# shehryar-malik/icrl

Measured on AMD Instinct MI355X. Metric: env-steps/sec (ICRL outer loop, HCWithPos-v0), higher is better.
Workload: dtype f32

## Files before the change

### icrl_amd/csrc/rollout.hip

```cpp
#include <stdio.h>
#include <stdlib.h>

#include "common.h"
#include "cost_fn.h"
#include "generic.h"

namespace icrl {

__global__ void policy_transpose_kernel(PolLayout L, const float* __restrict__ p, float* __restrict__ pt) {
  for (int i = blockIdx.x * blockDim.x + threadIdx.x; i < L.n; i += gridDim.x * blockDim.x) {
    int dst = i;
    for (int w = 0; w < 3; ++w) {
      if (i >= L.W1[w] && i < L.b1[w]) { int r = i - L.W1[w]; int j = r / L.O, k = r % L.O; dst = L.W1[w] + k * L.H1 + j; }
      if (i >= L.W2[w] && i < L.b2[w]) { int r = i - L.W2[w]; int j = r / L.H1, k = r % L.H1; dst = L.W2[w] + k * L.H2 + j; }
    }
    if (i >= L.Wa && i < L.ba) { int r = i - L.Wa; int a = r / L.H2, j = r % L.H2; dst = L.Wa + j * L.A + a; }
    pt[dst] = p[i];
  }
}

__global__ void costnet_transpose_kernel(CnLayout L, const float* __restrict__ p, float* __restrict__ pt) {
  for (int i = blockIdx.x * blockDim.x + threadIdx.x; i < L.n; i += gridDim.x * blockDim.x) {
    int dst = i;
    if (i >= L.W0 && i < L.b0) { int r = i - L.W0; int j = r / L.in, k = r % L.in; dst = L.W0 + k * L.H1 + j; }
// ... 10 lines not shown
  alignas(16) float x[MAX_OBS];
  alignas(16) float h[3][MAX_H];
  alignas(16) float g[3][MAX_H];
  alignas(16) float cx[MAX_CN_IN];
  alignas(16) float ch[2][MAX_H];
  float act_raw[MAX_ACT];
  float act_clip[MAX_ACT];
  float scal[4];
};

template <int OCT, int CIT>
struct WaveRegs {
  static constexpr int NA = 16 * (OCT > CIT ? OCT : CIT);
  union { float w1[NA]; float c0[NA]; };
  union { float w2[MAX_H]; float c1[MAX_H]; };
  float wh[MAX_H];
  union { float b1; float cb0; };
  union { float b2; float cb1; };
  union { float bh; float cbo; };
  union { float ls; float co; };
  float sd, lsd, i2v;
  int sel[(16 * (CIT > 0 ? CIT : 1) + WAVE - 1) / WAVE];
};
template <int OCT> using PolRegs = WaveRegs<OCT, 0>;
template <int CIT> using CnRegs = WaveRegs<0, CIT>;

template <int OCT, class Regs>
__device__ __forceinline__ void load_pol_regs(const PolLayout& L, const float* __restrict__ PT, Regs& R) {
  const int lane = threadIdx.x & 63;
  const int w = __builtin_amdgcn_readfirstlane(threadIdx.x >> 6);
  const int j1 = lane < L.H1 ? lane : 0, j2 = lane < L.H2 ? lane : 0;
#pragma unroll
  for (int k = 0; k < 16 * OCT; ++k) R.w1[k] = (w < 3 && k < L.O) ? PT[L.W1[w] + k * L.H1 + j1] : 0.f;
#pragma unroll
  for (int k = 0; k < MAX_H; ++k) R.w2[k] = (w < 3 && k < L.H1) ? PT[L.W2[w] + k * L.H2 + j2] : 0.f;
  R.b1 = w < 3 ? PT[L.b1[w] + j1] : 0.f;
  R.b2 = w < 3 ? PT[L.b2[w] + j2] : 0.f;
  R.bh = 0.f; R.ls = 0.f; R.sd = 1.f; R.lsd = 0.f; R.i2v = 2.f;
  if (w == 0) {
    const int a = lane < L.A ? lane : 0;
#pragma unroll
    for (int j = 0; j < MAX_H; ++j) R.wh[j] = j < L.H2 ? PT[L.Wa + j * L.A + a] : 0.f;
    R.bh = PT[L.ba + a];
    if (!L.discrete) R.ls = PT[L.log_std + a];
    R.sd = expf(R.ls); R.lsd = logf(R.sd); R.i2v = 2.f * (R.sd * R.sd);
  } else if (w < 3) {
#pragma unroll
    for (int j = 1; j < MAX_H; ++j) R.wh[j] = 0.f;
    R.wh[0] = PT[(w == 1 ? L.Wv : L.Wc) + j2];
    R.bh = PT[w == 1 ? L.bv : L.bc];
  }
}

template <int OCT, class Regs>
__device__ __forceinline__ void policy_forward_block(const PolLayout& L, const Regs& R, ActShared& sh,
                                                     const float* noise_row, int deterministic,
                                                     const float* alow, const float* ahigh,
                                                     const float* given = nullptr ) {
  const int lane = threadIdx.x & 63;
  const int w = __builtin_amdgcn_readfirstlane(threadIdx.x >> 6);
  if (w < 3) {
    f32x4 xs[4 * OCT];
#pragma unroll
    for (int i = 0; i < 4 * OCT; ++i) xs[i] = *reinterpret_cast<const f32x4*>(&sh.x[4 * i]);
    float acc = 0.f;
#pragma unroll
    for (int k = 0; k < 16 * OCT; ++k) acc = fmaf(R.w1[k], xs[k >> 2][k & 3], acc);
    sh.h[w][lane] = lane < L.H1 ? fast_tanh(acc + R.b1) : 0.f;
  }
  __syncthreads();
  if (w < 3) {
    f32x4 hs[MAX_H / 4];
#pragma unroll
    for (int i = 0; i < MAX_H / 4; ++i) hs[i] = *reinterpret_cast<const f32x4*>(&sh.h[w][4 * i]);
    float acc = 0.f;
#pragma unroll
    for (int k = 0; k < MAX_H; ++k) acc = fmaf(R.w2[k], hs[k >> 2][k & 3], acc);
    sh.g[w][lane] = lane < L.H2 ? fast_tanh(acc + R.b2) : 0.f;
  }
  __syncthreads();
  if (w == 0) {
    float mean = 0.f;
    {
      f32x4 gs[MAX_H / 4];
#pragma unroll
      for (int i = 0; i < MAX_H / 4; ++i) gs[i] = *reinterpret_cast<const f32x4*>(&sh.g[0][4 * i]);
      float acc = 0.f;
#pragma unroll
      for (int j = 0; j < MAX_H; ++j) acc = fmaf(R.wh[j], gs[j >> 2][j & 3], acc);
      mean = acc + R.bh;
    }
    if (!L.discrete) {
      float lp = 0.f, entl = 0.f;
      if (lane < L.A) {
        const float std = R.sd;
        float act = mean;
        if (given != nullptr) act = given[lane];
        else if (!deterministic) act = mean + noise_row[lane] * std;
        const float diff = act - mean;
        lp = -(diff * diff) / R.i2v - R.lsd - LOG_SQRT_2PI_F;
        entl = HALF_LOG_2PI_PLUS_HALF_F + R.lsd;
        sh.act_raw[lane] = act;
        float c = act;
        if (alow != nullptr && ahigh != nullptr) c = fminf(fmaxf(act, alow[lane]), ahigh[lane]);
        sh.act_clip[lane] = c;
      }
      lp = wave_sum_fast(lp);
      const float ent = wave_sum_fast(entl);
      if (lane == 0) { sh.scal[2] = lp; sh.scal[3] = ent; }
    } else {
      float m = wave_max(lane < L.A ? mean : -INFINITY);
      float e = lane < L.A ? expf(mean - m) : 0.f;
      float lse = m + logf(wave_sum(e));
      float logp = mean - lse;
      float p = lane < L.A ? expf(logp) : 0.f;
      float cdf = 0.f;
      int action = 0;
      if (given != nullptr) {
        action = (int)given[0];
      } else if (deterministic) {
        float best = wave_max(lane < L.A ? p : -1.f);
        unsigned long long ball = __ballot(lane < L.A && p == best);
        action = __ffsll((long long)ball) - 1;
      } else {
        const float u = noise_row[0];
        int cnt = 0;
        for (int a = 0; a < L.A; ++a) {
          cdf += __shfl(p, a, 64);
          cnt += (u >= cdf) ? 1 : 0;
        }
        action = cnt < L.A - 1 ? cnt : L.A - 1;
      }
      const float lp = __shfl(logp, action, 64);
// ... 618 lines not shown
    const int d = a.dones[n];
    if (d) nm.ret[n] = 0.0;
    if (has_cost) {
      double c = (double)a.raw_cost[n];
      if (nm.norm_cost) c = fmin(fmax(c / cden, -nm.clip_cost), nm.clip_cost);
      if (a.cost_out) a.cost_out[n] = c;
      if (a.cost_f32) a.cost_f32[n] = (float)c;
      if (d) nm.cost_ret[n] = 0.0;
    }
    if (a.last_dones) a.last_dones[n] = (uint8_t)d;
  }
}

__device__ __forceinline__ double np_pairwise_sum_wave(const double* a, int n) {
  const int leaves = n >> 7;
  if ((n & 127) != 0 || (leaves & (leaves - 1)) != 0 || leaves > 8) return np_pairwise_sum(a, n);
  const int lane = threadIdx.x & 63;
  const int L = lane >> 3, k = lane & 7;
  const double* p = a + 128 * (L < leaves ? L : 0) + k;
  double v[16];
#pragma unroll
  for (int i = 0; i < 16; ++i) v[i] = p[8 * i];
  double r = v[0];
#pragma unroll
  for (int i = 1; i < 16; ++i) r += v[i];
  r += __shfl_xor(r, 1, 64);
  r += __shfl_xor(r, 2, 64);
  r += __shfl_xor(r, 4, 64);
  if (leaves >= 2) r += __shfl_xor(r, 8, 64);
  if (leaves >= 4) r += __shfl_xor(r, 16, 64);
  if (leaves >= 8) r += __shfl_xor(r, 32, 64);
  return __shfl(r, 0, 64);
}

__device__ __forceinline__ double np_leaf_sum_wave(const double* a, int n) {
  const int lane = threadIdx.x & 63;
  if (n < 8) {
    double r = 0.0;
    for (int i = 0; i < n; ++i) r += a[i];
    return r;
  }
  double r = 0.0;
  if (lane < 8) {
    r = a[lane];
    for (int i = 8; i < n - (n % 8); i += 8) r += a[i + lane];
  }
  const double r0 = __shfl(r, 0, 64), r1 = __shfl(r, 1, 64), r2 = __shfl(r, 2, 64), r3 = __shfl(r, 3, 64);
  const double r4 = __shfl(r, 4, 64), r5 = __shfl(r, 5, 64), r6 = __shfl(r, 6, 64), r7 = __shfl(r, 7, 64);
  double res = ((r0 + r1) + (r2 + r3)) + ((r4 + r5) + (r6 + r7));
  for (int i = n - (n % 8); i < n; ++i) res += a[i];
  return res;
}

__device__ __forceinline__ void column_moments(const double* col, int stride, int N, double& bm, double& bv) {
  auto load16 = [&](int r0, double (&v)[16]) {
#pragma unroll
    for (int k = 0; k < 16; ++k) v[k] = col[(r0 + k < N ? r0 + k : N - 1) * stride];
  };
  double va[16], vb[16];
  double sum = 0.0;
  load16(0, va);
  for (int r0 = 0; r0 < N; r0 += 32) {
    load16(r0 + 16 < N ? r0 + 16 : 0, vb);
    __builtin_amdgcn_sched_barrier(0);
#pragma unroll
    for (int k = 0; k < 16; ++k) if (r0 + k < N) sum += va[k];
    load16(r0 + 32 < N ? r0 + 32 : 0, va);
    __builtin_amdgcn_sched_barrier(0);
#pragma unroll
    for (int k = 0; k < 16; ++k) if (r0 + 16 + k < N) sum += vb[k];
  }
  bm = sum / (double)N;
  double sq = 0.0;
  for (int r0 = 0; r0 < N; r0 += 32) {
    load16(r0 + 16 < N ? r0 + 16 : 0, vb);
#pragma unroll
    for (int k = 0; k < 16; ++k) { const double d = va[k] - bm; va[k] = d * d; }
    __builtin_amdgcn_sched_barrier(0);
#pragma unroll
    for (int k = 0; k < 16; ++k) if (r0 + k < N) sq += va[k];
    load16(r0 + 32 < N ? r0 + 32 : 0, va);
#pragma unroll
    for (int k = 0; k < 16; ++k) { const double d = vb[k] - bm; vb[k] = d * d; }
    __builtin_amdgcn_sched_barrier(0);
#pragma unroll
    for (int k = 0; k < 16; ++k) if (r0 + 16 + k < N) sq += vb[k];
  }
  bv = sq / (double)N;
}

__device__ __forceinline__ void column_moments_contig(const double* col, int N, double& bm, double& bv) {
  double va[16], vb[16];
  double sum = 0.0;
  const int NF = N & ~31;
#pragma unroll
  for (int k = 0; k < 16; ++k) va[k] = col[k];
  int r0 = 0;
  for (; r0 < NF; r0 += 32) {
#pragma unroll
    for (int k = 0; k < 16; ++k) vb[k] = col[r0 + 16 + k];
    __builtin_amdgcn_sched_barrier(0);
#pragma unroll
    for (int k = 0; k < 16; ++k) sum += va[k];
#pragma unroll
    for (int k = 0; k < 16; ++k) va[k] = col[r0 + 32 + k];
    __builtin_amdgcn_sched_barrier(0);
#pragma unroll
    for (int k = 0; k < 16; ++k) sum += vb[k];
  }
  if (r0 < N) {
#pragma unroll
    for (int k = 0; k < 16; ++k) vb[k] = col[r0 + 16 + k];
#pragma unroll
    for (int k = 0; k < 16; ++k) if (r0 + k < N) sum += va[k];
#pragma unroll
    for (int k = 0; k < 16; ++k) if (r0 + 16 + k < N) sum += vb[k];
  }
  bm = sum / (double)N;
  double sq = 0.0;
#pragma unroll
  for (int k = 0; k < 16; ++k) va[k] = col[k];
  for (r0 = 0; r0 < NF; r0 += 32) {
#pragma unroll
    for (int k = 0; k < 16; ++k) vb[k] = col[r0 + 16 + k];
#pragma unroll
    for (int k = 0; k < 16; ++k) { const double d = va[k] - bm; va[k] = d * d; }
    __builtin_amdgcn_sched_barrier(0);
#pragma unroll
    for (int k = 0; k < 16; ++k) sq += va[k];
#pragma unroll
    for (int k = 0; k < 16; ++k) va[k] = col[r0 + 32 + k];
#pragma unroll
    for (int k = 0; k < 16; ++k) { const double d = vb[k] - bm; vb[k] = d * d; }
    __builtin_amdgcn_sched_barrier(0);
#pragma unroll
    for (int k = 0; k < 16; ++k) sq += vb[k];
  }
  if (r0 < N) {
#pragma unroll
    for (int k = 0; k < 16; ++k) vb[k] = col[r0 + 16 + k];
#pragma unroll
    for (int k = 0; k < 16; ++k) { const double d = va[k] - bm; va[k] = d * d; }
#pragma unroll
    for (int k = 0; k < 16; ++k) { const double d = vb[k] - bm; vb[k] = d * d; }
#pragma unroll
    for (int k = 0; k < 16; ++k) if (r0 + k < N) sq += va[k];
#pragma unroll
    for (int k = 0; k < 16; ++k) if (r0 + 16 + k < N) sq += vb[k];
  }
  bv = sq / (double)N;
}

__global__ void __launch_bounds__(1024) norm_step_small_kernel(NormStepArgs a) {
  __shared__ double chunk[NORM_CHUNK];
  __shared__ double vec[2][128], dev2[2][128];
  __shared__ double mean_s[MAX_OBS], var_s[MAX_OBS];
  __shared__ double dens[2];
  const int tid = threadIdx.x, nt = blockDim.x, lane = tid & 63, wv = tid >> 6;
  const int N = a.N, O = a.O;
  const icrl_norm_t& nm = a.nm;
  const bool has_cost = a.raw_cost != nullptr;
  for (int i = tid; i < N * O; i += nt) chunk[i] = a.raw_obs[i];
  if (tid < N) {
    double r = nm.ret[tid], c = has_cost ? nm.cost_ret[tid] : 0.0;
    if (nm.training) {
      r = r * nm.reward_gamma + a.raw_rew[tid];
      if (has_cost) c = c * nm.cost_gamma + (double)a.raw_cost[tid];
    }
    vec[0][tid] = r; vec[1][tid] = c;
  }
  double o_mean = 0.0, o_var = 1.0, o_cnt = 0.0;
  if (tid < O) { o_mean = nm.obs_mean[tid]; o_var = nm.obs_var[tid]; o_cnt = nm.obs_count[0]; }
  __syncthreads();
  if (nm.training) {
    if (tid < O) {
      double bm, bv;
      column_moments(chunk + tid, O, N, bm, bv);
      chan_merge(o_mean, o_var, o_cnt, bm, bv, (double)N);
      nm.obs_mean[tid] = o_mean; nm.obs_var[tid] = o_var;
      if (tid == 0) nm.obs_count[0] = (double)N + o_cnt;
    }
    if (wv == 15 || (wv == 14 && has_cost)) {
      const int v = wv == 15 ? 0 : 1;
      double* st = v == 0 ? nm.ret_stats : nm.cost_stats;
      const double bm = np_leaf_sum_wave(vec[v], N) / (double)N;
      for (int i = lane; i < N; i += 64) { const double d = vec[v][i] - bm; dev2[v][i] = d * d; }
      __builtin_amdgcn_wave_barrier();
      __builtin_amdgcn_s_waitcnt(0xC07F);
      const double bv = np_leaf_sum_wave(dev2[v], N) / (double)N;
      double m = st[0], var = st[1];
      const double cnt = st[2];
      chan_merge(m, var, cnt, bm, bv, (double)N);
      if (lane == 0) { st[0] = m; st[1] = var; st[2] = (double)N + cnt; }
      if (lane == 0) dens[v] = sqrt(var + nm.epsilon);
    }
  } else {
    if (tid == 0) { dens[0] = sqrt(nm.ret_stats[1] + nm.epsilon); dens[1] = sqrt(nm.cost_stats[1] + nm.epsilon); }
  }
  if (nm.training && !has_cost && tid == 0) dens[1] = sqrt(nm.cost_stats[1] + nm.epsilon);
  if (tid < O) { mean_s[tid] = o_mean; var_s[tid] = o_var; }
  __syncthreads();
  for (int idx = tid; idx < N * O; idx += nt) {
    const int j = idx % O;
    double o = chunk[idx];
    if (nm.norm_obs) o = fmin(fmax((o - mean_s[j]) / sqrt(var_s[j] + nm.epsilon), -nm.clip_obs), nm.clip_obs);
    if (a.obs_out) a.obs_out[idx] = o;
    if (a.obs_f32) a.obs_f32[idx] = (float)o;
  }
  if (tid < N) {
    const int n = tid;
    double r = a.raw_rew[n];
    if (nm.norm_reward) r = fmin(fmax(r / dens[0], -nm.clip_reward), nm.clip_reward);
    if (a.rew_out) a.rew_out[n] = r;
    if (a.rew_f32) a.rew_f32[n] = (float)r;
    const int d = a.dones[n];
    if (nm.training || d) nm.ret[n] = d ? 0.0 : vec[0][n];
    if (has_cost) {
      double c = (double)a.raw_cost[n];
      if (nm.norm_cost) c = fmin(fmax(c / dens[1], -nm.clip_cost), nm.clip_cost);
      if (a.cost_out) a.cost_out[n] = c;
      if (a.cost_f32) a.cost_f32[n] = (float)c;
      if (nm.training || d) nm.cost_ret[n] = d ? 0.0 : vec[1][n];
    }
    if (a.last_dones) a.last_dones[n] = (uint8_t)d;
  }
}

constexpr int NORM_MAX_N_TRACE = 1024;
__device__ unsigned long long g_rollout_prof[8];
__device__ unsigned long long g_rollout_prof_wide[16];
__device__ unsigned long long g_wide_trace[NORM_MAX_N_TRACE * 4];
__device__ __forceinline__ unsigned long long prof_now() {
  unsigned long long t;
  asm volatile("s_memtime %0\n\ts_waitcnt lgkmcnt(0)" : "=s"(t)::"memory");
  return t;
}

struct PersistArgs {
  ActStepArgs act;
  icrl_norm_t nm;
  int T;
  double* xch_obs;
  double* xch_rew;
  float* xch_cost;
  unsigned* xch_done;
  unsigned* counter;
  unsigned long long* xg;
  unsigned g_magic;
  int prof;
};

__device__ __forceinline__ void xstore(double* p, double v) {
  __hip_atomic_store(reinterpret_cast<unsigned long long*>(p), (unsigned long long)__double_as_longlong(v), __ATOMIC_RELAXED, __HIP_MEMORY_SCOPE_AGENT);
}
__device__ __forceinline__ void xstore(float* p, float v) {
  __hip_atomic_store(reinterpret_cast<unsigned*>(p), __float_as_uint(v), __ATOMIC_RELAXED, __HIP_MEMORY_SCOPE_AGENT);
}
__device__ __forceinline__ void xstore(unsigned* p, unsigned v) { __hip_atomic_store(p, v, __ATOMIC_RELAXED, __HIP_MEMORY_SCOPE_AGENT); }
__device__ __forceinline__ double xload(const double* p) {
  return __longlong_as_double((long long)__hip_atomic_load(reinterpret_cast<const unsigned long long*>(p), __ATOMIC_RELAXED, __HIP_MEMORY_SCOPE_AGENT));
}
__device__ __forceinline__ float xload(const float* p) {
  return __uint_as_float(__hip_atomic_load(reinterpret_cast<const unsigned*>(p), __ATOMIC_RELAXED, __HIP_MEMORY_SCOPE_AGENT));
}
__device__ __forceinline__ unsigned xload(const unsigned* p) { return __hip_atomic_load(p, __ATOMIC_RELAXED, __HIP_MEMORY_SCOPE_AGENT); }
__device__ __forceinline__ void gstore(unsigned long long* p, unsigned tag, unsigned payload) {
  __hip_atomic_store(p, ((unsigned long long)tag << 32) | (unsigned long long)payload, __ATOMIC_RELAXED, __HIP_MEMORY_SCOPE_AGENT);
}
__device__ __forceinline__ unsigned long long gload(const unsigned long long* p) {
  return __hip_atomic_load(p, __ATOMIC_RELAXED, __HIP_MEMORY_SCOPE_AGENT);
}

__device__ __forceinline__ void grid_barrier(unsigned* flags, int N, int n, unsigned value, int& spin_limit) {
  asm volatile("s_waitcnt vmcnt(0)" ::: "memory");
  __syncthreads();
  if (threadIdx.x < 64) {
    const int lane = threadIdx.x;
    if (lane == 0) xstore(flags + n, value);
    int spins = 0;
    bool ok = false;
    while (spins < spin_limit && !ok) {
      const unsigned v0 = lane < N ? xload(flags + lane) : value;
      const unsigned v1 = lane + 64 < N ? xload(flags + lane + 64) : value;
      ok = __all(v0 >= value && v1 >= value);
      ++spins;
    }
    if (!ok) spin_limit = 1;
  }
  __syncthreads();
}

constexpr int GRAN_MAX = 12;
constexpr int REC_MAX = GRAN_MAX / 2;

static inline size_t persist_dyn_lds(int N, int O, int A) { return ((size_t)O * (size_t)(N + 64) + (size_t)O * (size_t)A) * sizeof(double); }

template <int OCT, int CIT, bool GRAN, bool PROF = false, bool MON = false, bool POINT = true, bool DISC = false>
__device__ __forceinline__ void rollout_persistent_body(const PersistArgs& p) {
  extern __shared__ __attribute__((aligned(16))) double dyn_lds[];
  __shared__ ActShared sh;
  double* const chunk = dyn_lds;
  double* const Bl = dyn_lds + p.act.pl.O * (p.act.env.n_envs + 64);
  __shared__ double vec[2][128], dev2[2][128], ret_s[128], cret_s[128], rawr_s[128];
  __shared__ float rawc_s[128];
  __shared__ double dens[2];
  __shared__ float noise_s[MAX_ACT], alow_s[MAX_ACT], ahigh_s[MAX_ACT];
  __shared__ int done_s[128];
  __shared__ int last_done_s;
  const ActStepArgs& a = p.act;
  icrl_norm_t nm = p.nm; globalize(nm);
  icrl_buffer_t buf = a.buf; globalize(buf);
  icrl_agent_t ag = a.ag; globalize(ag);
  icrl_costnet_t cnet = a.cn; globalize(cnet);
  unsigned long long* const xg_all = as_global(p.xg);
  const float* const noise_g = as_global(a.noise);
  double* const raw_plane = MON ? as_global(a.raw_plane) : nullptr;
  WaveRegs<OCT, CIT> R;
  WaveRegs<OCT, CIT>& C = R;
  load_pol_regs<OCT>(a.pl, a.PT, R);
  if constexpr (CIT > 0) { if (threadIdx.x >= 192 && a.has_cn) load_cn_regs<CIT>(a.cn, a.cl, C); }
  const icrl_cost_fn_t cf = a.cf;
  const int n = blockIdx.x;
  const int tid = threadIdx.x, lane = tid & 63;
  const int w = __builtin_amdgcn_readfirstlane(tid >> 6);
  const int O = a.pl.O, A = a.pl.A, N = a.env.n_envs, T = p.T;
  const int AS = buf.act_store;
  const int NA = a.pl.discrete ? 1 : A;
  const int NP = N + 64;
  const int G = 2 * O + 4;
  const int R16 = O + 2;
  typedef unsigned int rec_u4 __attribute__((ext_vector_type(4)));
  const __amdgpu_buffer_rsrc_t xrs = __builtin_amdgcn_make_buffer_rsrc(xg_all, 0, 2 * N * G * 8, 0x00020000);
  auto rstore = [&](int byte_off, rec_u4 v) { __builtin_amdgcn_raw_buffer_store_b128(v, xrs, byte_off, 0, 16); };
  auto rload = [&](int byte_off) -> rec_u4 { return __builtin_amdgcn_raw_buffer_load_b128(xrs, byte_off, 0, 16); };
  for (int i = tid; i < O * NP; i += 256) chunk[i] = 0.0;
  const bool has_cost = a.has_cn != 0;
  const uint32_t e_key = a.env.key[n];
  uint32_t e_ctr = a.env.step_count[n];
  int e_tep = a.env.t_ep[n];
  icrl_env_t env = a.env; globalize(env);
  for (int i = tid; i < O * a.env.act_dim; i += 256) Bl[i] = a.env.B[i];
  env.B = Bl;
  const bool has_box = a.alow != nullptr && a.ahigh != nullptr;
  if (tid < MAX_ACT) { alow_s[tid] = (has_box && tid < A) ? a.alow[tid] : 0.f; ahigh_s[tid] = (has_box && tid < A) ? a.ahigh[tid] : 0.f; }
  for (int i = tid; i < MAX_OBS; i += 256) {
    sh.x[i] = i < O ? (float)ag.last_obs[(size_t)n * O + i] : 0.f;
    if (i < O) sh.s_old[i] = a.env.s[(size_t)n * O + i];
  }
  if (tid < N) { ret_s[tid] = nm.ret[tid]; cret_s[tid] = nm.cost_ret[tid]; }
  if (tid == 0) last_done_s = ag.last_dones[n];
  double o_mean = 0.0, o_var = 1.0, o_cnt = 0.0, o_last = 0.0;
  if (tid < O) { o_mean = nm.obs_mean[tid]; o_var = nm.obs_var[tid]; o_cnt = nm.obs_count[0]; o_last = ag.last_obs[(size_t)n * O + tid]; }
  double st_m = 0.0, st_v = 1.0, st_c = 0.0;
  if (w == 3) { st_m = nm.ret_stats[0]; st_v = nm.ret_stats[1]; st_c = nm.ret_stats[2]; }
  if (w == 2) { st_m = nm.cost_stats[0]; st_v = nm.cost_stats[1]; st_c = nm.cost_stats[2]; }
  float noise_reg = (tid < NA) ? noise_g[(size_t)n * NA + tid] : 0.f;
  double fin_rew = 0.0; float fin_cost = 0.f; int fin_done = 0;
  unsigned long long pc0 = 0, pc1 = 0, pc2 = 0, pc3 = 0, pc4 = 0, pc5 = 0, pc_rounds = 0, tl = PROF ? prof_now() : 0ull;
  int spin_limit = 1 << 22;
  for (int t = 0; t < T; ++t) {
    const int par = t & 1;
    const size_t tn = (size_t)t * N + n;
    const unsigned gtag = (unsigned)(t + 1);
    if (tid < NA) {
      noise_s[tid] = noise_reg;
      if (t + 1 < T) noise_reg = noise_g[((size_t)(t + 1) * N + n) * NA + tid];
    }
    __syncthreads();
    policy_forward_block<OCT>(a.pl, R, sh, noise_s, 0, has_box ? alow_s : nullptr, has_box ? ahigh_s : nullptr);
    __syncthreads();
    if (w == 0) {
      double rew; int done;
      env_step_wave<POINT>(env, n, sh.s_old, sh.act_clip, e_key, e_ctr, e_tep, sh.s_new, rew, done);
      float* nob = buf.new_orig_observations + tn * O;
      if (GRAN) {
        const int rec0 = ((par * N + n) * R16) * 16;
        for (int i = lane; i < O; i += WAVE) {
          const double v = sh.s_new[i];
          nob[i] = (float)v;
          const unsigned long long bits = (unsigned long long)__double_as_longlong(v);
          rstore(rec0 + 16 * i, rec_u4{gtag, (unsigned)bits, (unsigned)(bits >> 32), gtag});
        }
        if (lane == 0) {
          const unsigned long long bits = (unsigned long long)__double_as_longlong(rew);
          rstore(rec0 + 16 * O, rec_u4{gtag, (unsigned)bits, (unsigned)(bits >> 32), gtag | (done ? 0x80000000u : 0u)});
        }
      } else {
        double* xo = as_global(p.xch_obs) + ((size_t)par * N + n) * O;
        for (int i = lane; i < O; i += WAVE) { const double v = sh.s_new[i]; nob[i] = (float)v; xstore(xo + i, v); }
        if (lane == 0) { xstore(as_global(p.xch_rew) + par * N + n, rew); xstore(as_global(p.xch_done) + par * N + n, (unsigned)done); }
      }
    } else if (w == 3) {
      float cost = 0.f;
      if constexpr (CIT == 0) cost = cost_fn_wave(cf, sh.s_old, sh.act_clip);
      else if (a.has_cn) cost = cost_forward_wave<CIT>(cnet, a.cl, C, sh.s_old, sh.act_clip, sh.cx, sh.ch, DISC ? 1 : 0);
      if (lane == 0) {
        if (GRAN) rstore(((par * N + n) * R16 + O + 1) * 16, rec_u4{gtag, __float_as_uint(cost), 0u, gtag});
        else xstore(as_global(p.xch_cost) + par * N + n, cost);
        buf.orig_costs[tn] = cost;
      }
    } else if (w == 2) {
      float* ob = buf.observations + tn * O;
      float* oob = buf.orig_observations + tn * O;
      for (int i = lane; i < O; i += WAVE) { ob[i] = sh.x[i]; oob[i] = (float)sh.s_old[i]; }
      if (lane < AS) buf.actions[tn * AS + lane] = sh.act_raw[lane];
      if (lane < A && !a.pl.discrete) ag.act_clipped[(size_t)n * A + lane] = sh.act_clip[lane];
      if (lane == 0) {
        buf.dones[tn] = (float)last_done_s;
        buf.reward_values[tn] = sh.scal[0];
        buf.cost_values[tn] = sh.scal[1];
        buf.log_probs[tn] = sh.scal[2];
        ag.last_v_r[n] = sh.scal[0];
        ag.last_v_c[n] = sh.scal[1];
      }
    }
    if (PROF) { const unsigned long long tn_ = prof_now(); pc0 += tn_ - tl; tl = tn_; }
    if (PROF && t == T / 2 && lane == 0) g_wide_trace[4 * n + w] = __builtin_amdgcn_s_memrealtime();
    if (GRAN) {
      const int rbase = par * N * R16 * 16;
      const int total = N * R16;
      rec_u4 g[REC_MAX];
#pragma unroll
      for (int k = 0; k < REC_MAX; ++k) g[k] = (k * 256 + tid < total) ? rload(rbase + (k * 256 + tid) * 16) : rec_u4{gtag, 0u, 0u, gtag};
      bool ok = false;
      int rounds = 0;
      for (int spins = 0; spins < spin_limit && !ok; ++spins) {
        ok = true;
#pragma unroll
        for (int k = 0; k < REC_MAX; ++k)
          if (g[k][0] != gtag || (g[k][3] & 0x7fffffffu) != gtag) { g[k] = rload(rbase + (k * 256 + tid) * 16); ok = false; }
        ++rounds;
      }
      if (PROF && tid == 0) { pc_rounds += (unsigned long long)rounds; }
      if (!ok) spin_limit = 1;
#pragma unroll
      for (int k = 0; k < REC_MAX; ++k) {
        const int idx = k * 256 + tid;
        if (idx < total) {
          unsigned rr = __umulhi((unsigned)idx, p.g_magic);
          int slot = idx - (int)rr * R16;
          if (slot >= R16) { slot -= R16; ++rr; }
          const double v = __longlong_as_double((long long)(((unsigned long long)g[k][2] << 32) | (unsigned long long)g[k][1]));
          if (slot < O) chunk[slot * NP + (int)rr] = v;
          else if (slot == O) { rawr_s[rr] = v; done_s[rr] = (int)(g[k][3] >> 31); }
          else rawc_s[rr] = has_cost ? __uint_as_float(g[k][1]) : 0.f;
        }
      }
      __syncthreads();
    } else {
      grid_barrier(as_global(p.counter), N, n, (unsigned)(t + 1), spin_limit);
    }
    if (PROF) { const unsigned long long tn_ = prof_now(); pc1 += tn_ - tl; tl = tn_; }
    {
      if (!GRAN) {
        const double* xo = as_global(p.xch_obs) + (size_t)par * N * O;
        for (int i = tid; i < N * O; i += 256) { const int rr = i / O, j = i - rr * O; chunk[j * NP + rr] = xload(xo + i); }
      }
      if (tid < N) {
        if (!GRAN) {
          rawr_s[tid] = xload(as_global(p.xch_rew) + par * N + tid);
          rawc_s[tid] = has_cost ? xload(as_global(p.xch_cost) + par * N + tid) : 0.f;
          done_s[tid] = (int)xload(as_global(p.xch_done) + par * N + tid);
        }
        const double rr = rawr_s[tid];
        const float rc = rawc_s[tid];
        double r = ret_s[tid], c = has_cost ? cret_s[tid] : 0.0;
        if (nm.training) {
          r = r * nm.reward_gamma + rr;
          if (has_cost) c = c * nm.cost_gamma + (double)rc;
        }
        vec[0][tid] = r; vec[1][tid] = c;
      }
    }
    __syncthreads();
    if (PROF) { const unsigned long long tn_ = prof_now(); pc3 += tn_ - tl; tl = tn_; }
    if (nm.training) {
      if (tid < O) {
        double bm, bv;
        column_moments_contig(chunk + tid * NP, N, bm, bv);
        chan_merge(o_mean, o_var, o_cnt, bm, bv, (double)N);
        o_cnt = (double)N + o_cnt;
      }
      if (w == 3 || (w == 2 && has_cost)) {
        const int v = w == 3 ? 0 : 1;
        const double bm = np_leaf_sum_wave(vec[v], N) / (double)N;
        for (int i = lane; i < N; i += 64) { const double d = vec[v][i] - bm; dev2[v][i] = d * d; }
        __builtin_amdgcn_wave_barrier();
        __builtin_amdgcn_s_waitcnt(0xC07F);
        const double bv = np_leaf_sum_wave(dev2[v], N) / (double)N;
        chan_merge(st_m, st_v, st_c, bm, bv, (double)N);
        st_c = (double)N + st_c;
      }
    }
    if (lane == 0 && w == 3) dens[0] = sqrt(st_v + nm.epsilon);
    if (lane == 0 && w == 2) dens[1] = sqrt(st_v + nm.epsilon);
    if (PROF) { const unsigned long long tn_ = prof_now(); pc4 += tn_ - tl; tl = tn_; }
    if (tid < O) {
      double o = chunk[tid * NP + n];
      if (nm.norm_obs) o = fmin(fmax((o - o_mean) / sqrt(o_var + nm.epsilon), -nm.clip_obs), nm.clip_obs);
      o_last = o;
      sh.x[tid] = (float)o;
      buf.new_observations[tn * O + tid] = (float)o;
      sh.s_old[tid] = sh.s_new[tid];
    }
    __syncthreads();
    if (PROF) { const unsigned long long tn_ = prof_now(); pc5 += tn_ - tl; tl = tn_; }
    if (tid < N) {
      const int d = done_s[tid];
      if (nm.training || d) { ret_s[tid] = d ? 0.0 : vec[0][tid]; if (has_cost) cret_s[tid] = d ? 0.0 : vec[1][tid]; }
    }
    if (tid == 0) {
      double r = rawr_s[n];
      fin_rew = r; fin_cost = rawc_s[n]; fin_done = done_s[n];
      if (nm.norm_reward) r = fmin(fmax(r / dens[0], -nm.clip_reward), nm.clip_reward);
      buf.rewards[tn] = (float)r;
      if (has_cost) {
        double c = (double)rawc_s[n];
        if (nm.norm_cost) c = fmin(fmax(c / dens[1], -nm.clip_cost), nm.clip_cost);
        buf.costs[tn] = (float)c;
      }
      last_done_s = done_s[n];
      if (MON) raw_plane[tn] = fin_rew;
    }
    if (PROF) { const unsigned long long tn_ = prof_now(); pc2 += tn_ - tl; tl = tn_; }
  }
  if (PROF && n == 0 && tid == 0) { g_rollout_prof[0] = pc0; g_rollout_prof[1] = pc1; g_rollout_prof[2] = pc2; g_rollout_prof[3] = (unsigned long long)T; g_rollout_prof[4] = pc3; g_rollout_prof[5] = pc4; g_rollout_prof[6] = pc5; g_rollout_prof[7] = pc_rounds; }
  if (spin_limit == 1 && ag.status != nullptr && (tid & 63) == 0) atomicOr(ag.status, 1);
  __syncthreads();
  if (tid < O) ag.last_obs[(size_t)n * O + tid] = o_last;
  if (tid == 0) {
    ag.last_dones[n] = (uint8_t)last_done_s;
    ag.raw_rew[n] = fin_rew; ag.dones[n] = (uint8_t)fin_done;
    if (has_cost) ag.raw_cost[n] = fin_cost;
  }
  if (n == 0) {
    if (tid < O) { nm.obs_mean[tid] = o_mean; nm.obs_var[tid] = o_var; }
    if (tid == 0) nm.obs_count[0] = o_cnt;
    if (lane == 0 && w == 3) { nm.ret_stats[0] = st_m; nm.ret_stats[1] = st_v; nm.ret_stats[2] = st_c; }
    if (lane == 0 && w == 2 && has_cost) { nm.cost_stats[0] = st_m; nm.cost_stats[1] = st_v; nm.cost_stats[2] = st_c; }
    if (tid < N) { nm.ret[tid] = ret_s[tid]; if (has_cost) nm.cost_ret[tid] = cret_s[tid]; }
  }
}

struct GenRolloutArgs {
  PersistArgs p;
  GenNet net;
  const float* P;
};
template <int OCT, int CIT, bool MON, bool DISC = false>
__device__ __forceinline__ void rollout_generic_body(const GenRolloutArgs& ga) {
  constexpr bool GRAN = true;
  const PersistArgs& p = ga.p;
  const GenNet& net = ga.net;
  __shared__ float gact[GEN_MAX_ROW];
  extern __shared__ __attribute__((aligned(16))) double dyn_lds[];
  __shared__ ActShared sh;
  double* const chunk = dyn_lds;
  double* const Bl = dyn_lds + p.act.pl.O * (p.act.env.n_envs + 64);
  __shared__ double vec[2][128], dev2[2][128], ret_s[128], cret_s[128], rawr_s[128];
  __shared__ float rawc_s[128];
  __shared__ double dens[2];
  __shared__ float noise_s[MAX_ACT], alow_s[MAX_ACT], ahigh_s[MAX_ACT];
  __shared__ int done_s[128];
  __shared__ int last_done_s;
  const ActStepArgs& a = p.act;
  icrl_norm_t nm = p.nm; globalize(nm);
  icrl_buffer_t buf = a.buf; globalize(buf);
  icrl_agent_t ag = a.ag; globalize(ag);
  icrl_costnet_t cnet = a.cn; globalize(cnet);
  unsigned long long* const xg_all = as_global(p.xg);
  const float* const noise_g = as_global(a.noise);
  double* const raw_plane = MON ? as_global(a.raw_plane) : nullptr;
  WaveRegs<OCT, CIT> R;
  WaveRegs<OCT, CIT>& C = R;
  if constexpr (CIT > 0) { if ((threadIdx.x >> 6) == 3 && a.has_cn) load_cn_regs<CIT>(a.cn, a.cl, C); }
  const icrl_cost_fn_t cf = a.cf;
  const int n = blockIdx.x;
  const int tid = threadIdx.x, lane = tid & 63;
  const int ctid = tid < 256 ? tid : (1 << 28);
  const float* const Pn = as_global(ga.P);
  const float* const PTn = as_global(a.PT);
  const int w = __builtin_amdgcn_readfirstlane(tid >> 6);
  const int O = a.pl.O, A = a.pl.A, N = a.env.n_envs, T = p.T;
  const int AS = buf.act_store;
  const int NA = a.pl.discrete ? 1 : A;
  const int NP = N + 64;
  const int G = 2 * O + 4;
  const int R16 = O + 2;
  typedef unsigned int rec_u4 __attribute__((ext_vector_type(4)));
  const __amdgpu_buffer_rsrc_t xrs = __builtin_amdgcn_make_buffer_rsrc(xg_all, 0, 2 * N * G * 8, 0x00020000);
  auto rstore = [&](int byte_off, rec_u4 v) { __builtin_amdgcn_raw_buffer_store_b128(v, xrs, byte_off, 0, 16); };
  auto rload = [&](int byte_off) -> rec_u4 { return __builtin_amdgcn_raw_buffer_load_b128(xrs, byte_off, 0, 16); };
  for (int i = ctid; i < O * NP; i += 256) chunk[i] = 0.0;
  const bool has_cost = a.has_cn != 0;
  const uint32_t e_key = a.env.key[n];
  uint32_t e_ctr = a.env.step_count[n];
  int e_tep = a.env.t_ep[n];
  icrl_env_t env = a.env; globalize(env);
  for (int i = ctid; i < O * a.env.act_dim; i += 256) Bl[i] = a.env.B[i];
  env.B = Bl;
  const bool has_box = a.alow != nullptr && a.ahigh != nullptr;
  if (tid < MAX_ACT) { alow_s[tid] = (has_box && tid < A) ? a.alow[tid] : 0.f; ahigh_s[tid] = (has_box && tid < A) ? a.ahigh[tid] : 0.f; }
  for (int i = ctid; i < MAX_OBS; i += 256) {
    sh.x[i] = i < O ? (float)ag.last_obs[(size_t)n * O + i] : 0.f;
    if (i < O) sh.s_old[i] = a.env.s[(size_t)n * O + i];
  }
  if (tid < N) { ret_s[tid] = nm.ret[tid]; cret_s[tid] = nm.cost_ret[tid]; }
  if (tid == 0) last_done_s = ag.last_dones[n];
  double o_mean = 0.0, o_var = 1.0, o_cnt = 0.0, o_last = 0.0;
  if (tid < O) { o_mean = nm.obs_mean[tid]; o_var = nm.obs_var[tid]; o_cnt = nm.obs_count[0]; o_last = ag.last_obs[(size_t)n * O + tid]; }
  double st_m = 0.0, st_v = 1.0, st_c = 0.0;
  if (w == 3) { st_m = nm.ret_stats[0]; st_v = nm.ret_stats[1]; st_c = nm.ret_stats[2]; }
  if (w == 2) { st_m = nm.cost_stats[0]; st_v = nm.cost_stats[1]; st_c = nm.cost_stats[2]; }
  float noise_reg = (tid < NA) ? noise_g[(size_t)n * NA + tid] : 0.f;
  double fin_rew = 0.0; float fin_cost = 0.f; int fin_done = 0;
  unsigned long long pc0 = 0, pc1 = 0, pc2 = 0, pc3 = 0, pc4 = 0, pc5 = 0, pc_rounds = 0, tl = p.prof ? prof_now() : 0ull;
  int spin_limit = 1 << 22;
  for (int t = 0; t < T; ++t) {
    const int par = t & 1;
    const size_t tn = (size_t)t * N + n;
    const unsigned gtag = (unsigned)(t + 1);
    if (tid < NA) {
      noise_s[tid] = noise_reg;
      if (t + 1 < T) noise_reg = noise_g[((size_t)(t + 1) * N + n) * NA + tid];
    }
    __syncthreads();
    gen_mlp_forward_quads(net, PTn, sh.x, gact, w, lane);
    if (tid == 0) {
      float lp, ent;
      gen_policy_head(net, Pn, gact + net.layer[net.head[0]].act_off, noise_s, 0, has_box ? alow_s : nullptr, has_box ? ahigh_s : nullptr, nullptr,
                      sh.act_raw, sh.act_clip, lp, ent);
      sh.scal[0] = gact[net.layer[net.head[1]].act_off]; sh.scal[1] = gact[net.layer[net.head[2]].act_off]; sh.scal[2] = lp;
    }
    __syncthreads();
    if (w == 0) {
      double rew; int done;
      env_step_wave(env, n, sh.s_old, sh.act_clip, e_key, e_ctr, e_tep, sh.s_new, rew, done);
      float* nob = buf.new_orig_observations + tn * O;
      if (GRAN) {
        const int rec0 = ((par * N + n) * R16) * 16;
        for (int i = lane; i < O; i += WAVE) {
          const double v = sh.s_new[i];
          nob[i] = (float)v;
          const unsigned long long bits = (unsigned long long)__double_as_longlong(v);
          rstore(rec0 + 16 * i, rec_u4{gtag, (unsigned)bits, (unsigned)(bits >> 32), gtag});
        }
        if (lane == 0) {
          const unsigned long long bits = (unsigned long long)__double_as_longlong(rew);
          rstore(rec0 + 16 * O, rec_u4{gtag, (unsigned)bits, (unsigned)(bits >> 32), gtag | (done ? 0x80000000u : 0u)});
        }
      } else {
        double* xo = as_global(p.xch_obs) + ((size_t)par * N + n) * O;
        for (int i = lane; i < O; i += WAVE) { const double v = sh.s_new[i]; nob[i] = (float)v; xstore(xo + i, v); }
        if (lane == 0) { xstore(as_global(p.xch_rew) + par * N + n, rew); xstore(as_global(p.xch_done) + par * N + n, (unsigned)done); }
      }
    } else if (w == 3) {
      float cost = 0.f;
      if constexpr (CIT == 0) cost = cost_fn_wave(cf, sh.s_old, sh.act_clip);
      else if (a.has_cn) cost = cost_forward_wave<CIT>(cnet, a.cl, C, sh.s_old, sh.act_clip, sh.cx, sh.ch, DISC ? 1 : 0);
      if (lane == 0) {
        if (GRAN) rstore(((par * N + n) * R16 + O + 1) * 16, rec_u4{gtag, __float_as_uint(cost), 0u, gtag});
        else xstore(as_global(p.xch_cost) + par * N + n, cost);
        buf.orig_costs[tn] = cost;
      }
    } else if (w == 2) {
      float* ob = buf.observations + tn * O;
      float* oob = buf.orig_observations + tn * O;
      for (int i = lane; i < O; i += WAVE) { ob[i] = sh.x[i]; oob[i] = (float)sh.s_old[i]; }
      if (lane < AS) buf.actions[tn * AS + lane] = sh.act_raw[lane];
      if (lane < A && !a.pl.discrete) ag.act_clipped[(size_t)n * A + lane] = sh.act_clip[lane];
      if (lane == 0) {
        buf.dones[tn] = (float)last_done_s;
        buf.reward_values[tn] = sh.scal[0];
        buf.cost_values[tn] = sh.scal[1];
        buf.log_probs[tn] = sh.scal[2];
        ag.last_v_r[n] = sh.scal[0];
        ag.last_v_c[n] = sh.scal[1];
      }
    }
    if (p.prof) { const unsigned long long tn_ = prof_now(); pc0 += tn_ - tl; tl = tn_; }
    if (p.prof && t == T / 2 && lane == 0) g_wide_trace[4 * n + w] = __builtin_amdgcn_s_memrealtime();
    if (GRAN) {
      const int rbase = par * N * R16 * 16;
      const int total = N * R16;
      rec_u4 g[REC_MAX];
#pragma unroll
      for (int k = 0; k < REC_MAX; ++k) g[k] = (k * 256 + ctid < total) ? rload(rbase + (k * 256 + ctid) * 16) : rec_u4{gtag, 0u, 0u, gtag};
      bool ok = false;
      int rounds = 0;
      for (int spins = 0; spins < spin_limit && !ok; ++spins) {
        ok = true;
#pragma unroll
        for (int k = 0; k < REC_MAX; ++k)
          if (g[k][0] != gtag || (g[k][3] & 0x7fffffffu) != gtag) { g[k] = rload(rbase + (k * 256 + ctid) * 16); ok = false; }
        ++rounds;
      }
      if (p.prof && tid == 0) { pc_rounds += (unsigned long long)rounds; }
      if (!ok) spin_limit = 1;
#pragma unroll
      for (int k = 0; k < REC_MAX; ++k) {
        const int idx = k * 256 + ctid;
        if (idx < total) {
          unsigned rr = __umulhi((unsigned)idx, p.g_magic);
          int slot = idx - (int)rr * R16;
          if (slot >= R16) { slot -= R16; ++rr; }
          const double v = __longlong_as_double((long long)(((unsigned long long)g[k][2] << 32) | (unsigned long long)g[k][1]));
          if (slot < O) chunk[slot * NP + (int)rr] = v;
          else if (slot == O) { rawr_s[rr] = v; done_s[rr] = (int)(g[k][3] >> 31); }
          else rawc_s[rr] = has_cost ? __uint_as_float(g[k][1]) : 0.f;
        }
      }
      __syncthreads();
    } else {
      grid_barrier(as_global(p.counter), N, n, (unsigned)(t + 1), spin_limit);
    }
    if (p.prof) { const unsigned long long tn_ = prof_now(); pc1 += tn_ - tl; tl = tn_; }
    {
      if (!GRAN) {
        const double* xo = as_global(p.xch_obs) + (size_t)par * N * O;
        for (int i = tid; i < N * O; i += 256) { const int rr = i / O, j = i - rr * O; chunk[j * NP + rr] = xload(xo + i); }
      }
      if (tid < N) {
        if (!GRAN) {
          rawr_s[tid] = xload(as_global(p.xch_rew) + par * N + tid);
          rawc_s[tid] = has_cost ? xload(as_global(p.xch_cost) + par * N + tid) : 0.f;
          done_s[tid] = (int)xload(as_global(p.xch_done) + par * N + tid);
        }
        const double rr = rawr_s[tid];
        const float rc = rawc_s[tid];
        double r = ret_s[tid], c = has_cost ? cret_s[tid] : 0.0;
        if (nm.training) {
          r = r * nm.reward_gamma + rr;
          if (has_cost) c = c * nm.cost_gamma + (double)rc;
        }
        vec[0][tid] = r; vec[1][tid] = c;
      }
    }
    __syncthreads();
    if (p.prof) { const unsigned long long tn_ = prof_now(); pc3 += tn_ - tl; tl = tn_; }
    if (nm.training) {
      if (tid < O) {
        double bm, bv;
        column_moments_contig(chunk + tid * NP, N, bm, bv);
        chan_merge(o_mean, o_var, o_cnt, bm, bv, (double)N);
        o_cnt = (double)N + o_cnt;
      }
      if (w == 3 || (w == 2 && has_cost)) {
        const int v = w == 3 ? 0 : 1;
        const double bm = np_leaf_sum_wave(vec[v], N) / (double)N;
        for (int i = lane; i < N; i += 64) { const double d = vec[v][i] - bm; dev2[v][i] = d * d; }
        __builtin_amdgcn_wave_barrier();
        __builtin_amdgcn_s_waitcnt(0xC07F);
        const double bv = np_leaf_sum_wave(dev2[v], N) / (double)N;
        chan_merge(st_m, st_v, st_c, bm, bv, (double)N);
        st_c = (double)N + st_c;
      }
    }
    if (lane == 0 && w == 3) dens[0] = sqrt(st_v + nm.epsilon);
    if (lane == 0 && w == 2) dens[1] = sqrt(st_v + nm.epsilon);
    if (p.prof) { const unsigned long long tn_ = prof_now(); pc4 += tn_ - tl; tl = tn_; }
    if (tid < O) {
      double o = chunk[tid * NP + n];
      if (nm.norm_obs) o = fmin(fmax((o - o_mean) / sqrt(o_var + nm.epsilon), -nm.clip_obs), nm.clip_obs);
      o_last = o;
      sh.x[tid] = (float)o;
      buf.new_observations[tn * O + tid] = (float)o;
      sh.s_old[tid] = sh.s_new[tid];
    }
    __syncthreads();
    if (p.prof) { const unsigned long long tn_ = prof_now(); pc5 += tn_ - tl; tl = tn_; }
    if (tid < N) {
      const int d = done_s[tid];
      if (nm.training || d) { ret_s[tid] = d ? 0.0 : vec[0][tid]; if (has_cost) cret_s[tid] = d ? 0.0 : vec[1][tid]; }
    }
    if (tid == 0) {
      double r = rawr_s[n];
      fin_rew = r; fin_cost = rawc_s[n]; fin_done = done_s[n];
      if (nm.norm_reward) r = fmin(fmax(r / dens[0], -nm.clip_reward), nm.clip_reward);
      buf.rewards[tn] = (float)r;
      if (has_cost) {
        double c = (double)rawc_s[n];
        if (nm.norm_cost) c = fmin(fmax(c / dens[1], -nm.clip_cost), nm.clip_cost);
        buf.costs[tn] = (float)c;
      }
      last_done_s = done_s[n];
      if (MON) raw_plane[tn] = fin_rew;
    }
    if (p.prof) { const unsigned long long tn_ = prof_now(); pc2 += tn_ - tl; tl = tn_; }
  }
  if (p.prof && n == 0 && tid == 0) { g_rollout_prof[0] = pc0; g_rollout_prof[1] = pc1; g_rollout_prof[2] = pc2; g_rollout_prof[3] = (unsigned long long)T; g_rollout_prof[4] = pc3; g_rollout_prof[5] = pc4; g_rollout_prof[6] = pc5; g_rollout_prof[7] = pc_rounds; }
  if (spin_limit == 1 && ag.status != nullptr && (tid & 63) == 0) atomicOr(ag.status, 1);
  __syncthreads();
  if (tid < O) ag.last_obs[(size_t)n * O + tid] = o_last;
  if (tid == 0) {
    ag.last_dones[n] = (uint8_t)last_done_s;
    ag.raw_rew[n] = fin_rew; ag.dones[n] = (uint8_t)fin_done;
    if (has_cost) ag.raw_cost[n] = fin_cost;
  }
  if (n == 0) {
    if (tid < O) { nm.obs_mean[tid] = o_mean; nm.obs_var[tid] = o_var; }
    if (tid == 0) nm.obs_count[0] = o_cnt;
    if (lane == 0 && w == 3) { nm.ret_stats[0] = st_m; nm.ret_stats[1] = st_v; nm.ret_stats[2] = st_c; }
    if (lane == 0 && w == 2 && has_cost) { nm.cost_stats[0] = st_m; nm.cost_stats[1] = st_v; nm.cost_stats[2] = st_c; }
    if (tid < N) { nm.ret[tid] = ret_s[tid]; if (has_cost) nm.cost_ret[tid] = cret_s[tid]; }
  }
}

template <int OCT, int CIT, bool MON = false>
__global__ void __launch_bounds__(256) rollout_generic_kernel(GenRolloutArgs ga) {
  rollout_generic_body<OCT, CIT, MON>(ga);
}

template <int OCT, int CIT, bool GRAN, bool PROF = false, bool MON = false>
__global__ void __launch_bounds__(256) rollout_persistent_kernel(PersistArgs p) {
  rollout_persistent_body<OCT, CIT, GRAN, PROF, MON, false>(p);
}

template <int OCT, int CIT, bool MON = false>
__global__ void __launch_bounds__(256) rollout_generic_disc_kernel(GenRolloutArgs ga) {
  rollout_generic_body<OCT, CIT, MON, true>(ga);
}
template <int OCT, int CIT, bool GRAN, bool MON = false>
__global__ void __launch_bounds__(256) rollout_persistent_disc_kernel(PersistArgs p) {
  rollout_persistent_body<OCT, CIT, GRAN, false, MON, false, true>(p);
}

// ... 3008 lines not shown
```

Baseline: 952,500.

## Replace block barriers with wave-local handoffs and fuse return-moment reductions

```diff
diff --git a/icrl_amd/csrc/rollout.hip b/icrl_amd/csrc/rollout.hip
--- a/icrl_amd/csrc/rollout.hip
+++ b/icrl_amd/csrc/rollout.hip
@@ -86,6 +86,11 @@
   }
 }
 
+__device__ __forceinline__ void layer_handoff() {
+  __builtin_amdgcn_wave_barrier();
+  __builtin_amdgcn_s_waitcnt(0xC07F);
+}
+
 template <int OCT, class Regs>
 __device__ __forceinline__ void policy_forward_block(const PolLayout& L, const Regs& R, ActShared& sh,
                                                      const float* noise_row, int deterministic,
@@ -102,7 +107,7 @@
     for (int k = 0; k < 16 * OCT; ++k) acc = fmaf(R.w1[k], xs[k >> 2][k & 3], acc);
     sh.h[w][lane] = lane < L.H1 ? fast_tanh(acc + R.b1) : 0.f;
   }
-  __syncthreads();
+  layer_handoff();
   if (w < 3) {
     f32x4 hs[MAX_H / 4];
 #pragma unroll
@@ -112,7 +117,7 @@
     for (int k = 0; k < MAX_H; ++k) acc = fmaf(R.w2[k], hs[k >> 2][k & 3], acc);
     sh.g[w][lane] = lane < L.H2 ? fast_tanh(acc + R.b2) : 0.f;
   }
-  __syncthreads();
+  layer_handoff();
   if (w == 0) {
     float mean = 0.f;
     {
@@ -837,6 +842,41 @@
   return res;
 }
 
+struct DivN {
+  double n, inv;
+  bool pow2;
+  __device__ __forceinline__ explicit DivN(int N, bool shortcut = true) : n((double)N), inv(1.0 / (double)N), pow2(shortcut && (N & (N - 1)) == 0) {}
+  __device__ __forceinline__ double operator()(double x) const { return pow2 ? x * inv : x / n; }
+};
+
+__device__ __forceinline__ void np_leaf_moments_wave(const double* a, double* dev2, int n, const DivN& over_n, double& bm, double& bv) {
+  const int lane = threadIdx.x & 63;
+  if (n >= 8 && (n & 7) == 0) {
+    const int nb = n >> 3;
+    double v[16];
+#pragma unroll
+    for (int k = 0; k < 16; ++k) v[k] = a[(k < nb ? 8 * k : 0) + (lane & 7)];
+    auto leaf = [&]() {
+      double r = v[0];
+#pragma unroll
+      for (int k = 1; k < 16; ++k) if (k < nb) r += v[k];
+      const double r0 = __shfl(r, 0, 64), r1 = __shfl(r, 1, 64), r2 = __shfl(r, 2, 64), r3 = __shfl(r, 3, 64);
+      const double r4 = __shfl(r, 4, 64), r5 = __shfl(r, 5, 64), r6 = __shfl(r, 6, 64), r7 = __shfl(r, 7, 64);
+      return ((r0 + r1) + (r2 + r3)) + ((r4 + r5) + (r6 + r7));
+    };
+    bm = over_n(leaf());
+#pragma unroll
+    for (int k = 0; k < 16; ++k) { const double d = v[k] - bm; v[k] = d * d; }
+    bv = over_n(leaf());
+    return;
+  }
+  bm = over_n(np_leaf_sum_wave(a, n));
+  for (int i = lane; i < n; i += 64) { const double d = a[i] - bm; dev2[i] = d * d; }
+  __builtin_amdgcn_wave_barrier();
+  __builtin_amdgcn_s_waitcnt(0xC07F);
+  bv = over_n(np_leaf_sum_wave(dev2, n));
+}
+
 __device__ __forceinline__ void column_moments(const double* col, int stride, int N, double& bm, double& bv) {
   auto load16 = [&](int r0, double (&v)[16]) {
 #pragma unroll
@@ -874,7 +914,7 @@
   bv = sq / (double)N;
 }
 
-__device__ __forceinline__ void column_moments_contig(const double* col, int N, double& bm, double& bv) {
+__device__ __forceinline__ void column_moments_contig(const double* col, int N, const DivN& over_n, double& bm, double& bv) {
   double va[16], vb[16];
   double sum = 0.0;
   const int NF = N & ~31;
@@ -901,7 +941,7 @@
 #pragma unroll
     for (int k = 0; k < 16; ++k) if (r0 + 16 + k < N) sum += vb[k];
   }
-  bm = sum / (double)N;
+  bm = over_n(sum);
   double sq = 0.0;
 #pragma unroll
   for (int k = 0; k < 16; ++k) va[k] = col[k];
@@ -933,7 +973,10 @@
 #pragma unroll
     for (int k = 0; k < 16; ++k) if (r0 + 16 + k < N) sq += vb[k];
   }
-  bv = sq / (double)N;
+  bv = over_n(sq);
+}
+__device__ __forceinline__ void column_moments_contig(const double* col, int N, double& bm, double& bv) {
+  column_moments_contig(col, N, DivN(N, false), bm, bv);
 }
 
 __global__ void __launch_bounds__(1024) norm_step_small_kernel(NormStepArgs a) {
@@ -1012,6 +1055,7 @@
 }
 
 constexpr int NORM_MAX_N_TRACE = 1024;
+constexpr int POLL_TRACE0 = 512;
 __device__ unsigned long long g_rollout_prof[8];
 __device__ unsigned long long g_rollout_prof_wide[16];
 __device__ unsigned long long g_wide_trace[NORM_MAX_N_TRACE * 4];
@@ -1092,6 +1136,7 @@
   __shared__ float noise_s[MAX_ACT], alow_s[MAX_ACT], ahigh_s[MAX_ACT];
   __shared__ int done_s[128];
   __shared__ int last_done_s;
+  __shared__ unsigned pub_s;
   const ActStepArgs& a = p.act;
   icrl_norm_t nm = p.nm; globalize(nm);
   icrl_buffer_t buf = a.buf; globalize(buf);
@@ -1142,7 +1187,13 @@
   float noise_reg = (tid < NA) ? noise_g[(size_t)n * NA + tid] : 0.f;
   double fin_rew = 0.0; float fin_cost = 0.f; int fin_done = 0;
   unsigned long long pc0 = 0, pc1 = 0, pc2 = 0, pc3 = 0, pc4 = 0, pc5 = 0, pc_rounds = 0, tl = PROF ? prof_now() : 0ull;
+  unsigned long long pw_rounds = 0, pw_early = 0;
+  if (PROF && tid == 0) pub_s = 0u;
   int spin_limit = 1 << 22;
+  const DivN over_n(N);
+  const bool ret_wave = w == 3 || (w == 2 && has_cost);
+  const int rv = w == 3 ? 0 : 1;
+  double* const rets = w == 3 ? ret_s : cret_s;
   for (int t = 0; t < T; ++t) {
     const int par = t & 1;
     const size_t tn = (size_t)t * N + n;
@@ -1170,6 +1221,7 @@
           const unsigned long long bits = (unsigned long long)__double_as_longlong(rew);
           rstore(rec0 + 16 * O, rec_u4{gtag, (unsigned)bits, (unsigned)(bits >> 32), gtag | (done ? 0x80000000u : 0u)});
         }
+        if (PROF && lane == 0) *(volatile unsigned*)&pub_s = gtag;
       } else {
         double* xo = as_global(p.xch_obs) + ((size_t)par * N + n) * O;
         for (int i = lane; i < O; i += WAVE) { const double v = sh.s_new[i]; nob[i] = (float)v; xstore(xo + i, v); }
@@ -1202,9 +1254,11 @@
     if (PROF) { const unsigned long long tn_ = prof_now(); pc0 += tn_ - tl; tl = tn_; }
     if (PROF && t == T / 2 && lane == 0) g_wide_trace[4 * n + w] = __builtin_amdgcn_s_memrealtime();
     if (GRAN) {
+      __syncthreads();
       const int rbase = par * N * R16 * 16;
       const int total = N * R16;
       rec_u4 g[REC_MAX];
+      if (PROF) { ++pw_rounds; pw_early += *(volatile unsigned*)&pub_s != gtag ? 1u : 0u; }
 #pragma unroll
       for (int k = 0; k < REC_MAX; ++k) g[k] = (k * 256 + tid < total) ? rload(rbase + (k * 256 + tid) * 16) : rec_u4{gtag, 0u, 0u, gtag};
       bool ok = false;
@@ -1215,6 +1269,7 @@
         for (int k = 0; k < REC_MAX; ++k)
           if (g[k][0] != gtag || (g[k][3] & 0x7fffffffu) != gtag) { g[k] = rload(rbase + (k * 256 + tid) * 16); ok = false; }
         ++rounds;
+        if (PROF && !ok) { ++pw_rounds; pw_early += *(volatile unsigned*)&pub_s != gtag ? 1u : 0u; }
       }
       if (PROF && tid == 0) { pc_rounds += (unsigned long long)rounds; }
       if (!ok) spin_limit = 1;
@@ -1241,38 +1296,34 @@
         const double* xo = as_global(p.xch_obs) + (size_t)par * N * O;
         for (int i = tid; i < N * O; i += 256) { const int rr = i / O, j = i - rr * O; chunk[j * NP + rr] = xload(xo + i); }
       }
-      if (tid < N) {
-        if (!GRAN) {
-          rawr_s[tid] = xload(as_global(p.xch_rew) + par * N + tid);
-          rawc_s[tid] = has_cost ? xload(as_global(p.xch_cost) + par * N + tid) : 0.f;
-          done_s[tid] = (int)xload(as_global(p.xch_done) + par * N + tid);
-        }
-        const double rr = rawr_s[tid];
-        const float rc = rawc_s[tid];
-        double r = ret_s[tid], c = has_cost ? cret_s[tid] : 0.0;
-        if (nm.training) {
-          r = r * nm.reward_gamma + rr;
-          if (has_cost) c = c * nm.cost_gamma + (double)rc;
-        }
-        vec[0][tid] = r; vec[1][tid] = c;
-      }
-    }
-    __syncthreads();
+      if (!GRAN && tid < N) {
+        rawr_s[tid] = xload(as_global(p.xch_rew) + par * N + tid);
+        rawc_s[tid] = has_cost ? xload(as_global(p.xch_cost) + par * N + tid) : 0.f;
+        done_s[tid] = (int)xload(as_global(p.xch_done) + par * N + tid);
+      }
+    }
+    if (!GRAN) __syncthreads();
+    if (ret_wave) {
+      for (int i = lane; i < N; i += 64) {
+        double r = rets[i];
+        if (nm.training) r = w == 3 ? r * nm.reward_gamma + rawr_s[i] : r * nm.cost_gamma + (double)rawc_s[i];
+        vec[rv][i] = r;
+      }
+      __builtin_amdgcn_wave_barrier();
+      __builtin_amdgcn_s_waitcnt(0xC07F);
+    }
     if (PROF) { const unsigned long long tn_ = prof_now(); pc3 += tn_ - tl; tl = tn_; }
     if (nm.training) {
       if (tid < O) {
         double bm, bv;
-        column_moments_contig(chunk + tid * NP, N, bm, bv);
+        column_moments_contig(chunk + tid * NP, N, over_n, bm, bv);
         chan_merge(o_mean, o_var, o_cnt, bm, bv, (double)N);
         o_cnt = (double)N + o_cnt;
       }
       if (w == 3 || (w == 2 && has_cost)) {
         const int v = w == 3 ? 0 : 1;
-        const double bm = np_leaf_sum_wave(vec[v], N) / (double)N;
-        for (int i = lane; i < N; i += 64) { const double d = vec[v][i] - bm; dev2[v][i] = d * d; }
-        __builtin_amdgcn_wave_barrier();
-        __builtin_amdgcn_s_waitcnt(0xC07F);
-        const double bv = np_leaf_sum_wave(dev2[v], N) / (double)N;
+        double bm, bv;
+        np_leaf_moments_wave(vec[v], dev2[v], N, over_n, bm, bv);
         chan_merge(st_m, st_v, st_c, bm, bv, (double)N);
         st_c = (double)N + st_c;
       }
@@ -1290,9 +1341,11 @@
     }
     __syncthreads();
     if (PROF) { const unsigned long long tn_ = prof_now(); pc5 += tn_ - tl; tl = tn_; }
-    if (tid < N) {
-      const int d = done_s[tid];
-      if (nm.training || d) { ret_s[tid] = d ? 0.0 : vec[0][tid]; if (has_cost) cret_s[tid] = d ? 0.0 : vec[1][tid]; }
+    if (ret_wave) {
+      for (int i = lane; i < N; i += 64) {
+        const int d = done_s[i];
+        if (nm.training || d) rets[i] = d ? 0.0 : vec[rv][i];
+      }
     }
     if (tid == 0) {
       double r = rawr_s[n];
@@ -1309,6 +1362,7 @@
     }
     if (PROF) { const unsigned long long tn_ = prof_now(); pc2 += tn_ - tl; tl = tn_; }
   }
+  if (PROF && lane == 0) { g_wide_trace[POLL_TRACE0 + 8 * n + 2 * w] = pw_rounds; g_wide_trace[POLL_TRACE0 + 8 * n + 2 * w + 1] = pw_early; }
   if (PROF && n == 0 && tid == 0) { g_rollout_prof[0] = pc0; g_rollout_prof[1] = pc1; g_rollout_prof[2] = pc2; g_rollout_prof[3] = (unsigned long long)T; g_rollout_prof[4] = pc3; g_rollout_prof[5] = pc4; g_rollout_prof[6] = pc5; g_rollout_prof[7] = pc_rounds; }
   if (spin_limit == 1 && ag.status != nullptr && (tid & 63) == 0) atomicOr(ag.status, 1);
   __syncthreads();
@@ -1401,6 +1455,10 @@
   double fin_rew = 0.0; float fin_cost = 0.f; int fin_done = 0;
   unsigned long long pc0 = 0, pc1 = 0, pc2 = 0, pc3 = 0, pc4 = 0, pc5 = 0, pc_rounds = 0, tl = p.prof ? prof_now() : 0ull;
   int spin_limit = 1 << 22;
+  const DivN over_n(N);
+  const bool ret_wave = w == 3 || (w == 2 && has_cost);
+  const int rv = w == 3 ? 0 : 1;
+  double* const rets = w == 3 ? ret_s : cret_s;
   for (int t = 0; t < T; ++t) {
     const int par = t & 1;
     const size_t tn = (size_t)t * N + n;
@@ -1466,6 +1524,7 @@
     if (p.prof) { const unsigned long long tn_ = prof_now(); pc0 += tn_ - tl; tl = tn_; }
     if (p.prof && t == T / 2 && lane == 0) g_wide_trace[4 * n + w] = __builtin_amdgcn_s_memrealtime();
     if (GRAN) {
+      __syncthreads();
       const int rbase = par * N * R16 * 16;
       const int total = N * R16;
       rec_u4 g[REC_MAX];
@@ -1505,38 +1564,34 @@
         const double* xo = as_global(p.xch_obs) + (size_t)par * N * O;
         for (int i = tid; i < N * O; i += 256) { const int rr = i / O, j = i - rr * O; chunk[j * NP + rr] = xload(xo + i); }
       }
-      if (tid < N) {
-        if (!GRAN) {
-          rawr_s[tid] = xload(as_global(p.xch_rew) + par * N + tid);
-          rawc_s[tid] = has_cost ? xload(as_global(p.xch_cost) + par * N + tid) : 0.f;
-          done_s[tid] = (int)xload(as_global(p.xch_done) + par * N + tid);
-        }
-        const double rr = rawr_s[tid];
-        const float rc = rawc_s[tid];
-        double r = ret_s[tid], c = has_cost ? cret_s[tid] : 0.0;
-        if (nm.training) {
-          r = r * nm.reward_gamma + rr;
-          if (has_cost) c = c * nm.cost_gamma + (double)rc;
-        }
-        vec[0][tid] = r; vec[1][tid] = c;
-      }
-    }
-    __syncthreads();
+      if (!GRAN && tid < N) {
+        rawr_s[tid] = xload(as_global(p.xch_rew) + par * N + tid);
+        rawc_s[tid] = has_cost ? xload(as_global(p.xch_cost) + par * N + tid) : 0.f;
+        done_s[tid] = (int)xload(as_global(p.xch_done) + par * N + tid);
+      }
+    }
+    if (!GRAN) __syncthreads();
+    if (ret_wave) {
+      for (int i = lane; i < N; i += 64) {
+        double r = rets[i];
+        if (nm.training) r = w == 3 ? r * nm.reward_gamma + rawr_s[i] : r * nm.cost_gamma + (double)rawc_s[i];
+        vec[rv][i] = r;
+      }
+      __builtin_amdgcn_wave_barrier();
+      __builtin_amdgcn_s_waitcnt(0xC07F);
+    }
     if (p.prof) { const unsigned long long tn_ = prof_now(); pc3 += tn_ - tl; tl = tn_; }
     if (nm.training) {
       if (tid < O) {
         double bm, bv;
-        column_moments_contig(chunk + tid * NP, N, bm, bv);
+        column_moments_contig(chunk + tid * NP, N, over_n, bm, bv);
         chan_merge(o_mean, o_var, o_cnt, bm, bv, (double)N);
         o_cnt = (double)N + o_cnt;
       }
       if (w == 3 || (w == 2 && has_cost)) {
         const int v = w == 3 ? 0 : 1;
-        const double bm = np_leaf_sum_wave(vec[v], N) / (double)N;
-        for (int i = lane; i < N; i += 64) { const double d = vec[v][i] - bm; dev2[v][i] = d * d; }
-        __builtin_amdgcn_wave_barrier();
-        __builtin_amdgcn_s_waitcnt(0xC07F);
-        const double bv = np_leaf_sum_wave(dev2[v], N) / (double)N;
+        double bm, bv;
+        np_leaf_moments_wave(vec[v], dev2[v], N, over_n, bm, bv);
         chan_merge(st_m, st_v, st_c, bm, bv, (double)N);
         st_c = (double)N + st_c;
       }
@@ -1554,9 +1609,11 @@
     }
     __syncthreads();
     if (p.prof) { const unsigned long long tn_ = prof_now(); pc5 += tn_ - tl; tl = tn_; }
-    if (tid < N) {
-      const int d = done_s[tid];
-      if (nm.training || d) { ret_s[tid] = d ? 0.0 : vec[0][tid]; if (has_cost) cret_s[tid] = d ? 0.0 : vec[1][tid]; }
+    if (ret_wave) {
+      for (int i = lane; i < N; i += 64) {
+        const int d = done_s[i];
+        if (nm.training || d) rets[i] = d ? 0.0 : vec[rv][i];
+      }
     }
     if (tid == 0) {
       double r = rawr_s[n];
```

Result: no change. 957,900 (median of 6 runs) (+0.6%).
